# ubi-agni/mujoco_ros_pkgs

Measured on AMD Instinct MI355X. Metric: env_steps_per_sec, higher is better.
Workload: dtype f64

## Files before the change

### mujoco_ros_pkgs_amd/csrc/lane_env_topos.h

```cpp
#pragma once

struct LeTopo_franka_like {
	static constexpr const char *name = "franka_like";
	static constexpr int NBODY = 12;
	static constexpr int NQ = 9;
	static constexpr int NV = 9;
	static constexpr int NU = 9;
	static constexpr int NA = 0;
	static constexpr int NJNT = 9;
	static constexpr int NSITE = 1;
	static constexpr int NSENSOR = 20;
	static constexpr int NSENSORDATA = 25;
	static constexpr int NM = 44;
	static constexpr int body_parentid[12] = { 0, 0, 1, 2, 3, 4, 5, 6, 7, 8, 9, 9 };
	static constexpr int body_rootid[12] = { 0, 1, 1, 1, 1, 1, 1, 1, 1, 1, 1, 1 };
	static constexpr int body_jnt[12] = { -1, -1, 0, 1, 2, 3, 4, 5, 6, -1, 7, 8 };
	static constexpr int body_sameframe[12] = { 1, 0, 0, 0, 0, 0, 0, 0, 0, 0, 0, 0 };
	static constexpr int body_gc[12] = { 0, 0, 0, 0, 0, 0, 0, 0, 0, 0, 0, 0 };
	static constexpr int jnt_type[9] = { 3, 3, 3, 3, 3, 3, 3, 2, 2 };
	static constexpr int jnt_bodyid[9] = { 2, 3, 4, 5, 6, 7, 8, 10, 11 };
	static constexpr int dof_parentid[9] = { -1, 0, 1, 2, 3, 4, 5, 6, 6 };
	static constexpr int dof_Madr[9] = { 0, 1, 3, 6, 10, 15, 21, 28, 36 };
	static constexpr int act_jnt[9] = { 0, 1, 2, 3, 4, 5, 6, 7, 8 };
	static constexpr int act_gaintype[9] = { 0, 0, 0, 0, 0, 0, 0, 0, 0 };
	static constexpr int act_biastype[9] = { 0, 0, 0, 0, 0, 0, 0, 0, 0 };
	static constexpr int act_ctrllimited[9] = { 1, 1, 1, 1, 1, 1, 1, 1, 1 };
	static constexpr int act_forcelimited[9] = { 0, 0, 0, 0, 0, 0, 0, 0, 0 };
	static constexpr int act_dyntype[9] = { 0, 0, 0, 0, 0, 0, 0, 0, 0 };
	static constexpr int act_actadr[9] = { 0, 0, 0, 0, 0, 0, 0, 0, 0 };
	static constexpr int act_actlimited[9] = { 0, 0, 0, 0, 0, 0, 0, 0, 0 };
	static constexpr int site_bodyid[1] = { 9 };
	static constexpr int site_sameframe[1] = { 0 };
	static constexpr int sensor_type[20] = { 8, 8, 8, 8, 8, 8, 8, 8, 8, 9, 9, 9, 9, 9, 9, 9, 9, 9, 23, 24 };
	static constexpr int sensor_objtype[20] = { 3, 3, 3, 3, 3, 3, 3, 3, 3, 3, 3, 3, 3, 3, 3, 3, 3, 3, 6, 6 };
	static constexpr int sensor_objid[20] = { 0, 1, 2, 3, 4, 5, 6, 7, 8, 0, 1, 2, 3, 4, 5, 6, 7, 8, 0, 0 };
	static constexpr int sensor_adr[20] = { 0, 1, 2, 3, 4, 5, 6, 7, 8, 9, 10, 11, 12, 13, 14, 15, 16, 17, 18, 21 };
};

struct LeTopo_lane_env_tree {
	static constexpr const char *name = "lane_env_tree";
	static constexpr int NBODY = 10;
	static constexpr int NQ = 8;
	static constexpr int NV = 8;
	static constexpr int NU = 7;
	static constexpr int NA = 0;
	static constexpr int NJNT = 8;
	static constexpr int NSITE = 2;
	static constexpr int NSENSOR = 12;
	static constexpr int NSENSORDATA = 24;
	static constexpr int NM = 17;
	static constexpr int body_parentid[10] = { 0, 0, 1, 2, 1, 4, 5, 5, 0, 8 };
	static constexpr int body_rootid[10] = { 0, 1, 1, 1, 1, 1, 1, 1, 8, 8 };
	static constexpr int body_jnt[10] = { -1, 0, 1, 2, -1, 3, 4, 5, 6, 7 };
	static constexpr int body_sameframe[10] = { 1, 1, 0, 0, 0, 0, 0, 0, 0, 0 };
	static constexpr int body_gc[10] = { 0, 0, 0, 0, 0, 0, 0, 0, 0, 0 };
	static constexpr int jnt_type[8] = { 3, 3, 2, 3, 3, 2, 3, 3 };
	static constexpr int jnt_bodyid[8] = { 1, 2, 3, 5, 6, 7, 8, 9 };
	static constexpr int dof_parentid[8] = { -1, 0, 1, 0, 3, 3, -1, 6 };
	static constexpr int dof_Madr[8] = { 0, 1, 3, 6, 8, 11, 14, 15 };
	static constexpr int act_jnt[7] = { 0, 1, 2, 3, 4, 5, 6 };
	static constexpr int act_gaintype[7] = { 0, 0, 0, 0, 0, 0, 0 };
	static constexpr int act_biastype[7] = { 0, 0, 1, 0, 0, 1, 0 };
	static constexpr int act_ctrllimited[7] = { 1, 1, 1, 0, 0, 0, 1 };
	static constexpr int act_forcelimited[7] = { 0, 0, 0, 1, 0, 0, 0 };
	static constexpr int act_dyntype[7] = { 0, 0, 0, 0, 0, 0, 0 };
	static constexpr int act_actadr[7] = { 0, 0, 0, 0, 0, 0, 0 };
	static constexpr int act_actlimited[7] = { 0, 0, 0, 0, 0, 0, 0 };
	static constexpr int site_bodyid[2] = { 3, 7 };
	static constexpr int site_sameframe[2] = { 0, 0 };
	static constexpr int sensor_type[12] = { 8, 9, 14, 12, 13, 23, 24, 23, 24, 23, 35, 8 };
	static constexpr int sensor_objtype[12] = { 3, 3, 18, 18, 18, 6, 6, 6, 1, 2, 0, 3 };
	static constexpr int sensor_objid[12] = { 1, 4, 2, 2, 5, 0, 0, 1, 6, 9, -1, 7 };
	static constexpr int sensor_adr[12] = { 0, 1, 2, 3, 4, 5, 8, 12, 15, 19, 22, 23 };
};

#define MJB_LE_TOPOS(X) X(0, LeTopo_franka_like) X(1, LeTopo_lane_env_tree)
#define MJB_LE_NTOPO 2
```

### mujoco_ros_pkgs_amd/csrc/mjb_lane_env.hip

```cpp
#include <hip/hip_runtime.h>

#include <dlfcn.h>
#include <sys/stat.h>
#include <unistd.h>

#include <cstdio>
#include <cstdlib>

#include <atomic>
#include <map>
#include <mutex>
#include <string>
#include <vector>

#include "mjb_lane_env_kernel.h"
#include "lane_env_topos.h"

namespace {

using namespace mjb_le;

template <class T, int LP, bool PE = false, bool HW = false, bool XF = false>
__global__ void __launch_bounds__(64) mjb_lane_env_kernel(const KernelParams MJB_AS4 *__restrict__ P, const int nsteps, const unsigned int step0,
                                                          const int env_lo, const int env_hi)
{
	extern __shared__ __attribute__((aligned(16))) unsigned char smem_le[];
	lane_env_body<T, LP, LE_SOLO, PE, HW, XF>(P, nsteps, step0, env_lo, env_hi, smem_le);
}

template <class T, int LP>
__global__ void __launch_bounds__(128) mjb_lane_env_duo_kernel(const KernelParams MJB_AS4 *__restrict__ P, const int nsteps, const unsigned int step0,
                                                               const int env_lo, const int env_hi)
{
	extern __shared__ __attribute__((aligned(16))) unsigned char smem_le[];
	lane_env_duo<T, LP>(P, nsteps, step0, env_lo, env_hi, smem_le);
}

template <class T>
__global__ void __launch_bounds__(128) mjb_lane_env_duo2_kernel(const KernelParams MJB_AS4 *__restrict__ P, const int nsteps, const unsigned int step0,
                                                                const int env_lo, const int env_hi)
{
	extern __shared__ __attribute__((aligned(16))) unsigned char smem_le[];
	lane_env_duo2<T, 160>(P, nsteps, step0, env_lo, env_hi, smem_le);
}

template <class T, int NW>
__global__ void __launch_bounds__(64 * NW) mjb_lane_env_trio_kernel(const KernelParams MJB_AS4 *__restrict__ P, const int nsteps, const unsigned int step0,
                                                                    const int env_lo, const int env_hi)
{
	extern __shared__ __attribute__((aligned(16))) unsigned char smem_le[];
	if constexpr (NW == 4) lane_env_quartet<T, 160>(P, nsteps, step0, env_lo, env_hi, smem_le);
	else lane_env_trio<T, 160>(P, nsteps, step0, env_lo, env_hi, smem_le);
}

template <class T> bool topo_matches(const mjb_model_desc &h)
{
	if (h.nbody != T::NBODY || h.nq != T::NQ || h.nv != T::NV || h.nu != T::NU || h.na != T::NA || h.njnt != T::NJNT || h.nsite != T::NSITE ||
	    h.nsensor != T::NSENSOR || h.nsensordata != T::NSENSORDATA || h.nM != T::NM)
		return false;
	for (int b = 0; b < h.nbody; b++) {
		const int jn = h.body_jntnum[b] == 1 ? h.body_jntadr[b] : -1;
		if (h.body_jntnum[b] > 1 || h.body_parentid[b] != T::body_parentid[b] || h.body_rootid[b] != T::body_rootid[b] || jn != T::body_jnt[b] ||
		    (h.body_sameframe[b] != 0) != (T::body_sameframe[b] != 0))
			return false;
	}
	for (int j = 0; j < h.njnt; j++)
		if (h.jnt_type[j] != T::jnt_type[j] || h.jnt_bodyid[j] != T::jnt_bodyid[j] || h.jnt_qposadr[j] != j || h.jnt_dofadr[j] != j) return false;
	for (int d = 0; d < h.nv; d++)
		if (h.dof_parentid[d] != T::dof_parentid[d] || h.dof_Madr[d] != T::dof_Madr[d] || h.dof_jntid[d] != d) return false;
	for (int i = 0; i < h.nu; i++)
		if (h.actuator_trntype[i] != MJB_TRN_JOINT || h.actuator_dyntype[i] != T::act_dyntype[i] || h.actuator_trnid[2 * i] != T::act_jnt[i] ||
		    h.actuator_gaintype[i] != T::act_gaintype[i] || h.actuator_biastype[i] != T::act_biastype[i] ||
		    (h.actuator_ctrllimited[i] != 0) != (T::act_ctrllimited[i] != 0) || (h.actuator_forcelimited[i] != 0) != (T::act_forcelimited[i] != 0) ||
		    (h.na > 0 && (h.actuator_actadr[i] != T::act_actadr[i] || (h.actuator_actlimited[i] != 0) != (T::act_actlimited[i] != 0))))
			return false;
	for (int i = 0; i < h.nsite; i++)
		if (h.site_bodyid[i] != T::site_bodyid[i] || (h.site_sameframe[i] != 0) != (T::site_sameframe[i] != 0)) return false;
	for (int i = 0; i < h.nsensor; i++)
		if (h.sensor_type[i] != T::sensor_type[i] || h.sensor_objtype[i] != T::sensor_objtype[i] || h.sensor_objid[i] != T::sensor_objid[i] ||
		    h.sensor_adr[i] != T::sensor_adr[i] || h.sensor_refid[i] >= 0)
			return false;
	return true;
}

}

static bool le_plain_tree(const mjb_model_desc *h)
{
	return h && h->nefcmax <= 0 && h->nconmax <= 0 && h->integrator == MJB_INT_EULER && h->nmocap <= 0 && h->ntendon <= 0 && h->neq <= 0 &&
	       h->nq == h->nv && h->njnt == h->nv;
}
static bool le_dyntype_ok(const mjb_model_desc *h, int i)
{
	const int d = h->actuator_dyntype[i];
	if (d == MJB_DYN_NONE) return h->na <= 0 || h->actuator_actadr[i] < 0;
	return (d == MJB_DYN_INTEGRATOR || d == MJB_DYN_FILTER) && h->actuator_actadr[i] >= 0 && h->actuator_actadr[i] < h->na;
}

int mjb_lane_env_match(const mjb_model_desc *h)
{
	if (!le_plain_tree(h)) return -1;
	for (int b = 1; b < h->nbody; b++)
		if (h->body_gravcomp[b] != 0) return -1;
#define MJB_LE_X(id, T) \
	if (topo_matches<T>(*h)) return id;
	MJB_LE_TOPOS(MJB_LE_X)
#undef MJB_LE_X
	return -1;
}

namespace {
struct LeVariant {
	int form;
	int sweep;
	int lds_kb;
	LeBuild build;
	int wave_lanes;
	const char *unavailable;
};
struct LeRow {
// ... 19 lines not shown
		if (r.form == form && r.sweep == sweep && r.build == build) return &r;
	return nullptr;
}
constexpr int le_block(const LeVariant &v) { return v.form == 3 ? 64 * v.sweep : (v.form ? 128 : v.wave_lanes); }
template <class T, int LP> constexpr int le_lds_bytes(int form, int sweep)
{
	return form == 3 ? (sweep == 4 ? quartet_bytes<T>() : trio_bytes<T>()) : (form == 2 ? duo2_bytes<T>() : (form == 1 ? duo_bytes<T, LP>() : Lds<T, LP>::bytes()));
}
}


int mjb_lane_env_eligible(const mjb_model_desc *h)
{
	if (!le_plain_tree(h) || h->nv < 1 || h->nbody > 24 || h->nv > 20) return 0;
	for (int j = 0; j < h->njnt; j++)
		if ((h->jnt_type[j] != MJB_JNT_SLIDE && h->jnt_type[j] != MJB_JNT_HINGE) || h->jnt_qposadr[j] != j || h->jnt_dofadr[j] != j || h->dof_jntid[j] != j) return 0;
	for (int b = 0; b < h->nbody; b++)
		if (h->body_jntnum[b] > 1) return 0;
	for (int i = 0; i < h->nsensor; i++) {
		const int t = h->sensor_type[i], ot = h->sensor_objtype[i];
		const bool frame = t == MJB_SENS_FRAMEPOS || t == MJB_SENS_FRAMEQUAT;
		if (!(frame || t == MJB_SENS_JOINTPOS || t == MJB_SENS_JOINTVEL || t == MJB_SENS_ACTUATORFRC || t == MJB_SENS_ACTUATORPOS || t == MJB_SENS_ACTUATORVEL ||
		      t == MJB_SENS_CLOCK))
			return 0;
		if (frame && (h->sensor_refid[i] >= 0 || (ot != MJB_OBJ_BODY && ot != MJB_OBJ_XBODY && ot != MJB_OBJ_SITE))) return 0;
	}
	for (int i = 0; i < h->nu; i++)
		if (h->actuator_trntype[i] != MJB_TRN_JOINT || !le_dyntype_ok(h, i)) return 0;
	int owned = 0;
	for (int i = 0; i < h->nu; i++) owned += h->actuator_dyntype[i] != MJB_DYN_NONE;
	return owned == (h->na > 0 ? h->na : 0);
}

namespace {

std::string topo_source(const mjb_model_desc &h)
{
	std::string s = "struct LeTopo_rt {\n";
	auto scalar = [&](const char *n, int v) { s += std::string("\tstatic constexpr int ") + n + " = " + std::to_string(v) + ";\n"; };
	auto arr = [&](const char *n, int count, auto get) {
		s += std::string("\tstatic constexpr int ") + n + "[" + std::to_string(count > 0 ? count : 1) + "] = { ";
		for (int i = 0; i < (count > 0 ? count : 1); i++) s += (i ? ", " : "") + std::to_string(count > 0 ? (int)get(i) : 0);
		s += " };\n";
	};
	scalar("NBODY", h.nbody); scalar("NQ", h.nq); scalar("NV", h.nv); scalar("NU", h.nu); scalar("NA", h.na); scalar("NJNT", h.njnt); scalar("NSITE", h.nsite);
	scalar("NSENSOR", h.nsensor); scalar("NSENSORDATA", h.nsensordata); scalar("NM", h.nM);
	arr("body_parentid", h.nbody, [&](int i) { return h.body_parentid[i]; });
	arr("body_rootid", h.nbody, [&](int i) { return h.body_rootid[i]; });
	arr("body_jnt", h.nbody, [&](int i) { return h.body_jntnum[i] == 1 ? h.body_jntadr[i] : -1; });
	arr("body_sameframe", h.nbody, [&](int i) { return h.body_sameframe[i] != 0; });
	arr("body_gc", h.nbody, [&](int i) { return i > 0 && h.body_gravcomp[i] != 0; });
	arr("jnt_type", h.njnt, [&](int i) { return h.jnt_type[i]; });
	arr("jnt_bodyid", h.njnt, [&](int i) { return h.jnt_bodyid[i]; });
	arr("dof_parentid", h.nv, [&](int i) { return h.dof_parentid[i]; });
	arr("dof_Madr", h.nv, [&](int i) { return h.dof_Madr[i]; });
	arr("act_jnt", h.nu, [&](int i) { return h.actuator_trnid[2 * i]; });
	arr("act_gaintype", h.nu, [&](int i) { return h.actuator_gaintype[i]; });
	arr("act_biastype", h.nu, [&](int i) { return h.actuator_biastype[i]; });
	arr("act_ctrllimited", h.nu, [&](int i) { return h.actuator_ctrllimited[i] != 0; });
	arr("act_forcelimited", h.nu, [&](int i) { return h.actuator_forcelimited[i] != 0; });
	arr("act_dyntype", h.nu, [&](int i) { return h.actuator_dyntype[i]; });
	arr("act_actadr", h.nu, [&](int i) { return h.na > 0 ? h.actuator_actadr[i] : 0; });
	arr("act_actlimited", h.nu, [&](int i) { return h.na > 0 && h.actuator_actlimited[i] != 0; });
	arr("site_bodyid", h.nsite, [&](int i) { return h.site_bodyid[i]; });
	arr("site_sameframe", h.nsite, [&](int i) { return h.site_sameframe[i] != 0; });
	arr("sensor_type", h.nsensor, [&](int i) { return h.sensor_type[i]; });
	arr("sensor_objtype", h.nsensor, [&](int i) { return h.sensor_objtype[i]; });
	arr("sensor_objid", h.nsensor, [&](int i) { return h.sensor_objid[i]; });
	arr("sensor_adr", h.nsensor, [&](int i) { return h.sensor_adr[i]; });
	s += "};\n";
	return s;
}

struct RtcApi {
	void *lib = nullptr;
	int (*create)(void **, const char *, const char *, int, const char **, const char **) = nullptr;
	int (*compile)(void *, int, const char **) = nullptr;
	int (*log_size)(void *, size_t *) = nullptr;
	int (*log)(void *, char *) = nullptr;
	int (*code_size)(void *, size_t *) = nullptr;
	int (*code)(void *, char *) = nullptr;
	int (*destroy)(void **) = nullptr;
	bool ok = false;
};
RtcApi &rtc()
{
	static RtcApi a = [] {
		RtcApi r;
		for (const char *n : { "libhiprtc.so", "libhiprtc.so.7", "/opt/rocm/lib/libhiprtc.so" }) {
			r.lib = dlopen(n, RTLD_NOW | RTLD_LOCAL);
			if (r.lib) break;
		}
		if (!r.lib) return r;
		r.create = (decltype(r.create))dlsym(r.lib, "hiprtcCreateProgram");
		r.compile = (decltype(r.compile))dlsym(r.lib, "hiprtcCompileProgram");
		r.log_size = (decltype(r.log_size))dlsym(r.lib, "hiprtcGetProgramLogSize");
		r.log = (decltype(r.log))dlsym(r.lib, "hiprtcGetProgramLog");
		r.code_size = (decltype(r.code_size))dlsym(r.lib, "hiprtcGetCodeSize");
		r.code = (decltype(r.code))dlsym(r.lib, "hiprtcGetCode");
		r.destroy = (decltype(r.destroy))dlsym(r.lib, "hiprtcDestroyProgram");
		r.ok = r.create && r.compile && r.log_size && r.log && r.code_size && r.code && r.destroy;
		return r;
	}();
	return a;
}

// ... 529 lines not shown
```

### mujoco_ros_pkgs_amd/csrc/mjb_lane_env_kernel.h

```cpp
#pragma once
#ifndef __HIPCC_RTC__
#include <hip/hip_runtime.h>
#endif

#include "mjb_dev.h"
#include "mjb_math.h"

namespace mjb_le {

template <int V> struct IC {
	static constexpr int value = V;
	constexpr operator int() const { return V; }
};
template <int... Is> struct ISeq {};
template <int N, int... Is> struct MkSeq : MkSeq<N - 1, N - 1, Is...> {};
template <int... Is> struct MkSeq<0, Is...> { using type = ISeq<Is...>; };
template <typename F, int... Is> DEVI void sfor_impl(F &&f, ISeq<Is...>) { (f(IC<Is>{}), ...); }
template <int N, typename F> DEVI void sfor(F &&f) { sfor_impl(f, typename MkSeq<N>::type{}); }

DEVI double frcp(double x)
{
	double r = __builtin_amdgcn_rcp(x);
	r = fma(fma(-x, r, 1.0), r, r);
	r = fma(fma(-x, r, 1.0), r, r);
// ... 168 lines not shown
template <class T, int LP> struct Lds {
	using Q = Tq<T>;
	static constexpr bool needed(int b)
	{
		for (int a = b; a > 0; a = T::body_parentid[a])
			if (T::body_jnt[a] >= 0) return true;
		return false;
	}
	static constexpr int slot(int b)
	{
		int n = 0;
		for (int a = 1; a < b; a++)
			if (needed(a)) n++;
		return T::NV + 3 * n;
	}
	static constexpr int cin_slot(int b)
	{
		int at = slot(T::NBODY);
		for (int a = T::NBODY - 1; a >= 1; a--) {
			if (!needed(a)) continue;
			if (at + 5 > LP) return -1;
			if (a == b) return at;
			at += 5;
		}
		return -1;
	}
	static constexpr int nmov() { return (slot(T::NBODY) - T::NV) / 3; }
	static constexpr int nslots() { return le_solo_slots(T::NV, nmov(), LP); }
	static constexpr int bytes() { return nslots() * LE_SLOT_BYTES; }
};

struct alignas(16) Pair { double a, b; };

template <class T> struct PeSlots {
	static constexpr bool moving(int b) { return Lds<T, (1 << 20)>::needed(b); }
	static constexpr int njb(int b) { int n = 0; for (int a = 1; a < b; a++) if (T::body_jnt[a] >= 0) n++; return n; }
	static constexpr int nmb(int b) { int n = 0; for (int a = 1; a < b; a++) if (moving(a)) n++; return n; }
	static constexpr int gravity(int k) { return k; }
	static constexpr int joint(int b, int f) { return 3 + 4 * njb(b) + f; }
	static constexpr int inert(int b, int f) { return 3 + 4 * njb(T::NBODY) + 7 * nmb(b) + f; }
	static constexpr int act(int i, int f) { return 3 + 4 * njb(T::NBODY) + 7 * nmb(T::NBODY) + 6 * i + f; }
	static constexpr int rest(int b) { return act(T::NU, 0) + (b - 1 - nmb(b)); }
	static constexpr int n = act(T::NU, 0) + (T::NBODY - 1 - nmb(T::NBODY));
};

template <class T> struct XfSlots {
	static constexpr int slot(int b) { return PeSlots<T>::nmb(b); }
	static constexpr int n = PeSlots<T>::nmb(T::NBODY);
};

template <class T, class = void> struct LeGc { static constexpr bool on(int) { return false; } };
template <class T> struct LeGc<T, decltype((void)T::body_gc)> { static constexpr bool on(int b) { return T::body_gc[b] != 0; } };
template <class T> constexpr bool le_any_gc() { for (int b = 1; b < T::NBODY; b++) if (LeGc<T>::on(b)) return true; return false; }

enum LeRole : int {
	LE_SOLO = 0,
	LE_DUO_P = 1,
	LE_DUO_V = 2,
	LE_PIPE_P = 3,
	LE_PIPE_V = 4,
	LE_TRIO_P = 5,
	LE_TRIO_C = 6,
	LE_TRIO_V = 7,
	LE_QUAD_O = 8,
	LE_QUAD_X = 9,
	LE_QUAD_C = 10,
	LE_QUAD_V = 11,
};
constexpr bool le_two_halves(int role) { return role == LE_DUO_P || role == LE_DUO_V; }
constexpr bool le_pipelined_duo(int role) { return role == LE_PIPE_P || role == LE_PIPE_V; }
constexpr bool le_trio(int role) { return role == LE_TRIO_P || role == LE_TRIO_C || role == LE_TRIO_V; }
constexpr bool le_quartet(int role) { return role == LE_QUAD_O || role == LE_QUAD_X || role == LE_QUAD_C || role == LE_QUAD_V; }
DEVI void le_barrier() { asm volatile("s_waitcnt lgkmcnt(0)\n\ts_barrier" ::: "memory"); }
template <int NV> struct DuoSlots { static constexpr int n = le_exchange_slots(NV); };
template <class T, int LP, int ROLE = LE_SOLO, bool PE = false, bool HW = false, bool XF = false>
DEVI void lane_env_body(const KernelParams MJB_AS4 *__restrict__ P, const int nsteps, const unsigned int step0, const int env_lo, const int env_hi,
                        unsigned char *const smem_le)
{
	constexpr int NB = T::NBODY, NV = T::NV, NU = T::NU, NA = T::NA;
	constexpr bool QUAD = le_quartet(ROLE), TRIQ = le_trio(ROLE) || QUAD;
	constexpr bool HALVES = ROLE == LE_SOLO || le_two_halves(ROLE);
	constexpr bool DP = ROLE == LE_SOLO || ROLE == LE_DUO_P || ROLE == LE_PIPE_P || ROLE == LE_TRIO_C || ROLE == LE_QUAD_C, DV = ROLE == LE_SOLO || ROLE == LE_DUO_V || ROLE == LE_PIPE_V || ROLE == LE_TRIO_V || ROLE == LE_QUAD_V, DUO = ROLE != LE_SOLO;
	constexpr bool PIPE = le_pipelined_duo(ROLE) || TRIQ;
	constexpr bool POSE = HALVES || ROLE == LE_PIPE_P || ROLE == LE_TRIO_P, RINGC = ROLE == LE_PIPE_V || ROLE == LE_TRIO_C || ROLE == LE_TRIO_V;
	constexpr bool VLDS = ROLE == LE_TRIO_V || ROLE == LE_QUAD_V;
	constexpr bool EPOS = ROLE == LE_SOLO || ROLE == LE_DUO_P || ROLE == LE_PIPE_P || ROLE == LE_TRIO_P || ROLE == LE_QUAD_X;
	constexpr bool SENSF = ROLE == LE_SOLO || ROLE == LE_DUO_V || ROLE == LE_PIPE_P || ROLE == LE_TRIO_P || ROLE == LE_QUAD_X;
	[[maybe_unused]] constexpr bool XW = ROLE == LE_QUAD_X;
	[[maybe_unused]] constexpr bool DPW = DP || XW;
	[[maybe_unused]] constexpr bool FM = ROLE != LE_QUAD_C, FH = !XW;
	[[maybe_unused]] constexpr bool POSEW = ROLE == LE_TRIO_P || ROLE == LE_QUAD_X;
	[[maybe_unused]] constexpr bool OWNCIN = ROLE != LE_TRIO_V;
	using Q = Tq<T>;
	static_assert(!PE || ROLE == LE_SOLO, "lane = env kernel: per-env overrides run the solo form");
	static_assert(!HW || (ROLE == LE_SOLO && !PE), "lane = env kernel: the hwsim stage runs the solo form, without per-env overrides");
	static_assert(!XF || (ROLE == LE_SOLO && !HW), "lane = env kernel: xfrc_applied runs the solo form, without the hwsim stage");
	static_assert(NA == 0 || (ROLE == LE_SOLO && !HW), "lane = env kernel: activation states run the solo form, without the hwsim stage");
	static_assert(!le_any_gc<T>() || ROLE == LE_SOLO, "lane = env kernel: gravity compensation runs the solo form");
	using OV = PeSlots<T>;
	using XS6 = XfSlots<T>;
	constexpr int LPE = PIPE ? (1 << 20) : (DUO ? LP - DuoSlots<NV>::n : LP);
	using LD = Lds<T, LPE>;
	static_assert(LD::slot(T::NBODY) <= LPE, "lane = env kernel: state and forces of the topology need more LDS than this instantiation's budget");
	constexpr auto SCUSE = [](int b) {
		if (b < 3 || b >= T::NBODY || T::body_jnt[b] < 0) return false;
		if (T::jnt_type[T::body_jnt[b]] != MJB_JNT_HINGE) return false;
// ... 266 lines not shown
						matvec3(v, xm, ip);
						for (int k = 0; k < 3; k++) dif[k] += v[k];
					}
					const double mass = tj.mass;
					const double *X = xm;
					const double ixx = tj.ibody[0], iyy = tj.ibody[1], izz = tj.ibody[2], ixy = tj.ibody[3], ixz = tj.ibody[4], iyz = tj.ibody[5];
					double Tm[9];
					for (int rr = 0; rr < 3; rr++) {
						Tm[3 * rr + 0] = X[3 * rr] * ixx + X[3 * rr + 1] * ixy + X[3 * rr + 2] * ixz;
						Tm[3 * rr + 1] = X[3 * rr] * ixy + X[3 * rr + 1] * iyy + X[3 * rr + 2] * iyz;
						Tm[3 * rr + 2] = X[3 * rr] * ixz + X[3 * rr + 1] * iyz + X[3 * rr + 2] * izz;
					}
					ci[0] = Tm[0] * X[0] + Tm[1] * X[1] + Tm[2] * X[2] + mass * (dif[1] * dif[1] + dif[2] * dif[2]);
					ci[1] = Tm[3] * X[3] + Tm[4] * X[4] + Tm[5] * X[5] + mass * (dif[0] * dif[0] + dif[2] * dif[2]);
					ci[2] = Tm[6] * X[6] + Tm[7] * X[7] + Tm[8] * X[8] + mass * (dif[0] * dif[0] + dif[1] * dif[1]);
					ci[3] = Tm[0] * X[3] + Tm[1] * X[4] + Tm[2] * X[5] - mass * dif[0] * dif[1];
					ci[4] = Tm[0] * X[6] + Tm[1] * X[7] + Tm[2] * X[8] - mass * dif[0] * dif[2];
					ci[5] = Tm[3] * X[6] + Tm[4] * X[7] + Tm[5] * X[8] - mass * dif[1] * dif[2];
					ci[6] = mass * dif[0];
					ci[7] = mass * dif[1];
					ci[8] = mass * dif[2];
					ci[9] = mass;
					if constexpr (OWNCIN) for (int k = 0; k < 5; k++) lp[64 * (c0 + k)] = Pair{ ci[2 * k], ci[2 * k + 1] };
				}
				[[maybe_unused]] double pv[6], pa[6];
				if constexpr (!DV) {
				} else if constexpr (p == 0 || !LD::needed(p)) {
					for (int k = 0; k < 6; k++) pv[k] = 0;
					pa[0] = pa[1] = pa[2] = 0;
					for (int k = 0; k < 3; k++) pa[3 + k] = -grav[k];
				} else {
					for (int k = 0; k < 6; k++) { pv[k] = cvel[p][k]; pa[k] = cacc[p][k]; }
				}
				if constexpr (j >= 0) {
					[[maybe_unused]] double qv = 0;
					if constexpr (DV) qv = lp[64 * j].b;
					double *cd = cdof[j];
					constexpr int cq = CD0 + 3 * (ord % 2);
					if constexpr (ROLE == LE_QUAD_V) {
						const Pair d0 = lp[64 * cq], d1 = lp[64 * (cq + 1)], d2 = lp[64 * (cq + 2)];
						cd[0] = d0.a; cd[1] = d0.b; cd[2] = d1.a; cd[3] = d1.b; cd[4] = d2.a; cd[5] = d2.b;
						if constexpr (T::jnt_type[j] == MJB_JNT_SLIDE) cd[0] = cd[1] = cd[2] = 0;
					} else {
					const LeTapeBody MJB_AS4 &tj = tb[b];
					const double ax[3] = { tj.jaxis[0], tj.jaxis[1], tj.jaxis[2] };
					double xaxis[3];
					matvec3(xaxis, xm, ax);
					if constexpr (T::jnt_type[j] == MJB_JNT_SLIDE) {
						cd[0] = cd[1] = cd[2] = 0;
						for (int k = 0; k < 3; k++) cd[3 + k] = xaxis[k];
					} else {
						const double jp[3] = { tj.jpos[0], tj.jpos[1], tj.jpos[2] };
						double xanch[3] = { xp[0], xp[1], xp[2] }, off[3];
						if (jp[0] != 0 || jp[1] != 0 || jp[2] != 0) {
							double v[3];
							matvec3(v, xm, jp);
							for (int k = 0; k < 3; k++) xanch[k] += v[k];
						}
						for (int k = 0; k < 3; k++) off[k] = -xanch[k];
						for (int k = 0; k < 3; k++) cd[k] = xaxis[k];
						cross3(cd + 3, xaxis, off);
					}
					if constexpr (ROLE == LE_QUAD_C) {
						lp[64 * cq] = Pair{ cd[0], cd[1] };
						lp[64 * (cq + 1)] = Pair{ cd[2], cd[3] };
						lp[64 * (cq + 2)] = Pair{ cd[4], cd[5] };
					}
					}
					if constexpr (!DV) {
					} else if constexpr (p == 0 || !LD::needed(p)) {
						for (int k = 0; k < 6; k++) { cvel[b][k] = cd[k] * qv; cacc[b][k] = pa[k]; }
					} else {
						double cdd[6];
						cross_motion(cdd, pv, cd);
						for (int k = 0; k < 6; k++) { cvel[b][k] = pv[k] + cd[k] * qv; cacc[b][k] = pa[k] + cdd[k] * qv; }
					}
				} else if constexpr (DV) {
					for (int k = 0; k < 6; k++) { cvel[b][k] = pv[k]; cacc[b][k] = pa[k]; }
				}
				if constexpr (DV) {
					double cf[6], t0[6], t1[6];
					mul_inert_vec(cf, ci, cacc[b]);
					mul_inert_vec(t0, ci, cvel[b]);
					cross_force(t1, cvel[b], t0);
					constexpr int q0 = LD::slot(b);
					lp[64 * q0] = Pair{ cf[0] + t1[0], cf[1] + t1[1] };
					lp[64 * (q0 + 1)] = Pair{ cf[2] + t1[2], cf[3] + t1[3] };
					lp[64 * (q0 + 2)] = Pair{ cf[4] + t1[4], cf[5] + t1[5] };
				}
			};
			[[maybe_unused]] double hcmd[NV > 0 ? NV : 1], hpi[NV > 0 ? NV : 1], hpl[NV > 0 ? NV : 1], hjp[NV > 0 ? NV : 1], hjv[NV > 0 ? NV : 1], hlu = 0, hlw = 0;
			[[maybe_unused]] auto hw_fetch = [&]() __attribute__((always_inline)) {
				if (Pq->hw.period_ns > 0) {
					const double *const cad = Pq->hw.cad + ev * (size_t)(2 + 2 * Pq->hw.n);
					hlu = cad[0];
					hlw = cad[1];
				}
				sfor<NV>([&](auto I) __attribute__((always_inline)) {
					hcmd[I] = hpi[I] = hpl[I] = hjp[I] = hjv[I] = 0;
					const HwSim MJB_AS4 &hw = Pq->hw;
					const int k = hw.le_tab[4 * I];
					if (k >= 0) {
						const int method = hw.le_tab[4 * I + 1], hn = hw.n;
						const size_t at = ev * (size_t)hn + (size_t)k;
						if (method == MJB_HW_EFFORT) hcmd[I] = hw.cmd_eff[at];
						else if (method == MJB_HW_VELOCITY || method == MJB_HW_VELOCITY_PID) hcmd[I] = hw.cmd_vel[at];
						else if (hw.estop != 0) hcmd[I] = hw.cmd_hold[at];
// ... 227 lines not shown
						}
						constexpr int q0 = LD::slot(b);
						lp[64 * q0] = Pair{ cf[0] + t1[0], cf[1] + t1[1] };
						lp[64 * (q0 + 1)] = Pair{ cf[2] + t1[2], cf[3] + t1[3] };
						lp[64 * (q0 + 2)] = Pair{ cf[4] + t1[4], cf[5] + t1[5] };
					}
					if constexpr (ROLE == LE_PIPE_P || ROLE == LE_TRIO_P) {
						constexpr int ord = (LD::slot(b) - NV) / 3, rg = RING + 6 * (ord % RINGN);
						const double *xm = xmat[b];
						double xp[3] = { 0, 0, 0 };
						if constexpr (r != b) for (int k = 0; k < 3; k++) xp[k] = xpos[b][k] - xpos[r][k];
						lp[64 * rg] = Pair{ xp[0], xp[1] };
						lp[64 * (rg + 1)] = Pair{ xp[2], xm[0] };
						lp[64 * (rg + 2)] = Pair{ xm[1], xm[2] };
						lp[64 * (rg + 3)] = Pair{ xm[3], xm[4] };
						lp[64 * (rg + 4)] = Pair{ xm[5], xm[6] };
						lp[64 * (rg + 5)] = Pair{ xm[7], xm[8] };
						LE_PK(0);
						le_barrier();
						LE_PK(2);
					}
				}
				if constexpr (b + 1 < NB) touch_rec<14>(hA[b + 1]);
				if constexpr (DV && b == NB - 1) sfor<NV>([&](auto I) { qfa[I] = s.qfrc_applied[ev * NV + I]; });
				if constexpr (HW && b == NB - 1) hw_fetch();
				__builtin_amdgcn_sched_barrier(0);
				}
			});


			if constexpr (QUAD) {
				constexpr auto HINGE = [](int c) {
					if (c < 1 || c >= T::NBODY || T::body_jnt[c < T::NBODY ? (c < 0 ? 0 : c) : 0] < 0) return false;
					return T::jnt_type[T::body_jnt[c]] == MJB_JNT_HINGE;
				};
				constexpr auto NEXTN = [](int c) { for (int q = c + 1; q < T::NBODY; q++) if (LD::needed(q)) return q; return T::NBODY; };
				constexpr auto NTH = [](int k) { int c = 0; for (int i = 0; i < k && c < T::NBODY; i++) { c++; while (c < T::NBODY && !LD::needed(c)) c++; } return k < 1 ? T::NBODY : c; };
				constexpr int KN = [] { int n = 0; for (int c = 1; c < T::NBODY; c++) if (LD::needed(c)) n++; return n; }();
				constexpr int N1 = NEXTN(0), N2 = NEXTN(N1 < NB ? N1 : NB - 1);
				[[maybe_unused]] double osn[NB + 1], ocs[NB + 1], oq0[NB + 1];
				[[maybe_unused]] Pair opq[NB + 1];
				auto o_body = [&](auto Bq) {
					constexpr int b = Bq;
					constexpr int p = T::body_parentid[b], j = T::body_jnt[b];
					const double *const A = hA[b];
					constexpr int qr = QR0 + 4 * (((LD::slot(b) - NV) / 3) % 2);
					double quat[4] = { A[3], A[4], A[5], A[6] };
					if constexpr (p != 0) {
						double q[4];
						qmul(q, xquat[p], quat);
						for (int k = 0; k < 4; k++) quat[k] = q[k];
					}
					if constexpr (j >= 0) {
						if (A[10] != 0 || A[11] != 0 || A[12] != 0) {
							lp[64 * (qr + 2)] = Pair{ quat[0], quat[1] };
							lp[64 * (qr + 3)] = Pair{ quat[2], quat[3] };
						}
						if constexpr (T::jnt_type[j] == MJB_JNT_HINGE) {
							double ql[4], q[4];
							ql[0] = ocs[b]; ql[1] = A[7] * osn[b]; ql[2] = A[8] * osn[b]; ql[3] = A[9] * osn[b];
							qmul(q, quat, ql);
							for (int k = 0; k < 4; k++) quat[k] = q[k];
						}
					}
					normalize4_sel(quat);
					for (int k = 0; k < 4; k++) xquat[b][k] = quat[k];
					if constexpr (LD::needed(b)) {
						lp[64 * qr] = Pair{ quat[0], quat[1] };
						lp[64 * (qr + 1)] = Pair{ quat[2], quat[3] };
					}
				};
				auto o_phase = [&](auto Bq) {
					constexpr int b = Bq, nx = NEXTN(b), nx2 = NEXTN(nx < NB ? nx : NB - 1);
					touch_s(hA[b][0]);
					if constexpr (nx < NB) for (int k = 0; k < 14; k++) hA[nx][k] = reinterpret_cast<const double MJB_AS4 *>(tb + nx)[k];
					if constexpr (nx < NB && HINGE(nx2)) {
						opq[nx2] = lp[64 * T::body_jnt[nx2 < NB ? nx2 : 0]];
						oq0[nx2] = tb[nx2].qpos0;
					}
					if constexpr (HINGE(nx)) sincos_nb((opq[nx].a - oq0[nx]) * 0.5, &osn[nx], &ocs[nx]);
					o_body(Bq);
					if constexpr (nx < NB) touch_rec<14>(hA[nx]);
				};
				auto x_body = [&](auto Bq) {
					constexpr int b = Bq;
					constexpr int p = T::body_parentid[b], j = T::body_jnt[b], r = T::body_rootid[b];
					constexpr int qr = QR0 + 4 * (((LD::slot(b) - NV) / 3) % 2);
					const double *const A = hA[b];
					double pos[3] = { A[0], A[1], A[2] }, quat[4] = { A[3], A[4], A[5], A[6] };
					if constexpr (LD::needed(b)) {
						const Pair g0 = lp[64 * qr], g1 = lp[64 * (qr + 1)];
						quat[0] = g0.a; quat[1] = g0.b; quat[2] = g1.a; quat[3] = g1.b;
					} else {
						if constexpr (p != 0) {
							double q[4];
							qmul(q, xquat[p], quat);
							for (int k = 0; k < 4; k++) quat[k] = q[k];
						}
						normalize4_sel(quat);
					}
					[[maybe_unused]] Pair sp{ 0, 0 };
					if constexpr (j >= 0) sp = lp[64 * j];
					if constexpr (p != 0) {
						double v[3];
						matvec3(v, xmat[p], pos);
						for (int k = 0; k < 3; k++) pos[k] = v[k] + xpos[p][k];
					}
					[[maybe_unused]] double xanch[3], qp = 0;
					[[maybe_unused]] bool offc = false;
					if constexpr (j >= 0) {
						qp = sp.a;
						const double jp[3] = { A[10], A[11], A[12] };
						offc = jp[0] != 0 || jp[1] != 0 || jp[2] != 0;
						for (int k = 0; k < 3; k++) xanch[k] = pos[k];
						if (offc) {
							const Pair h0 = lp[64 * (qr + 2)], h1 = lp[64 * (qr + 3)];
							const double q0[4] = { h0.a, h0.b, h1.a, h1.b };
							double M0[9], v[3];
							quat2mat_nocheck(M0, q0);
							matvec3(v, M0, jp);
							for (int k = 0; k < 3; k++) xanch[k] += v[k];
						}
						if (ep_on && pas_on) {
							const double dqs = qp - tb[b].spring;
							pe += 0.5 * tb[b].stiffness * dqs * dqs;
						}
					}
					for (int k = 0; k < 4; k++) xquat[b][k] = quat[k];
					quat2mat_nocheck(xmat[b], quat);
					if constexpr (j >= 0) {
						if constexpr (T::jnt_type[j] == MJB_JNT_SLIDE) {
							const double ax[3] = { A[7], A[8], A[9] };
							double xaxis[3];
							matvec3(xaxis, xmat[b], ax);
							const double dq = qp - A[13];
							for (int k = 0; k < 3; k++) pos[k] += xaxis[k] * dq;
						} else if (offc) {
							const double jp[3] = { A[10], A[11], A[12] };
							double v[3];
							matvec3(v, xmat[b], jp);
							for (int k = 0; k < 3; k++) pos[k] = xanch[k] - v[k];
						}
					}
					for (int k = 0; k < 3; k++) xpos[b][k] = pos[k];
					const double *const Bh = hB[b];
					double xipos[3];
					if constexpr (T::body_sameframe[b]) {
						for (int k = 0; k < 3; k++) xipos[k] = xpos[b][k];
					} else {
						double ip[3] = { Bh[0], Bh[1], Bh[2] }, v[3];
						matvec3(v, xmat[b], ip);
						for (int k = 0; k < 3; k++) xipos[k] = v[k] + xpos[b][k];
					}
					if (eg_on) pe -= Bh[9] * (grav[0] * xipos[0] + grav[1] * xipos[1] + grav[2] * xipos[2]);
					frame_sensors(Bq, xipos);
					if constexpr (LD::needed(b)) {
						constexpr int ord = (LD::slot(b) - NV) / 3, rg = RING + 6 * (ord % RINGN);
						const double *xm = xmat[b];
						double xp[3] = { 0, 0, 0 };
						if constexpr (r != b) for (int k = 0; k < 3; k++) xp[k] = xpos[b][k] - xpos[r][k];
						lp[64 * rg] = Pair{ xp[0], xp[1] };
						lp[64 * (rg + 1)] = Pair{ xp[2], xm[0] };
						lp[64 * (rg + 2)] = Pair{ xm[1], xm[2] };
						lp[64 * (rg + 3)] = Pair{ xm[3], xm[4] };
						lp[64 * (rg + 4)] = Pair{ xm[5], xm[6] };
						lp[64 * (rg + 5)] = Pair{ xm[7], xm[8] };
						if constexpr (j >= 0) {
							double *cd = cdof[j];
							const double ax[3] = { A[7], A[8], A[9] };
							double xaxis[3];
							matvec3(xaxis, xm, ax);
							if constexpr (T::jnt_type[j] == MJB_JNT_SLIDE) {
								cd[0] = cd[1] = cd[2] = 0;
								for (int k = 0; k < 3; k++) cd[3 + k] = xaxis[k];
							} else {
								const double jp[3] = { A[10], A[11], A[12] };
								double xa[3] = { xp[0], xp[1], xp[2] }, off[3];
								if (jp[0] != 0 || jp[1] != 0 || jp[2] != 0) {
									double v[3];
									matvec3(v, xm, jp);
									for (int k = 0; k < 3; k++) xa[k] += v[k];
								}
								for (int k = 0; k < 3; k++) off[k] = -xa[k];
								for (int k = 0; k < 3; k++) cd[k] = xaxis[k];
								cross3(cd + 3, xaxis, off);
							}
						}
					}
				};
				auto x_phase = [&](auto Bq) {
					constexpr int b = Bq, nx = NEXTN(b);
					touch_s(hA[b][0]);
					touch_s(hB[b][0]);
					if constexpr (nx < NB) {
						for (int k = 0; k < 14; k++) hA[nx][k] = reinterpret_cast<const double MJB_AS4 *>(tb + nx)[k];
						for (int k = 0; k < 10; k++) hB[nx][k] = reinterpret_cast<const double MJB_AS4 *>(tb + nx)[16 + k];
					}
					x_body(Bq);
					if constexpr (nx < NB) {
						touch_rec<14>(hA[nx]);
						touch_rec<10>(hB[nx]);
					}
				};
				if constexpr (ROLE == LE_QUAD_O || ROLE == LE_QUAD_X) {
					sfor<NB>([&](auto Bq) {
						constexpr int b = Bq;
						if constexpr (b > 0 && !LD::needed(b)) {
							for (int k = 0; k < 14; k++) hA[b][k] = reinterpret_cast<const double MJB_AS4 *>(tb + b)[k];
							if constexpr (ROLE == LE_QUAD_X) for (int k = 0; k < 10; k++) hB[b][k] = reinterpret_cast<const double MJB_AS4 *>(tb + b)[16 + k];
							if constexpr (ROLE == LE_QUAD_O) o_body(Bq);
							else x_body(Bq);
						}
					});
					if constexpr (N1 < NB) {
						for (int k = 0; k < 14; k++) hA[N1][k] = reinterpret_cast<const double MJB_AS4 *>(tb + N1)[k];
						if constexpr (ROLE == LE_QUAD_X) for (int k = 0; k < 10; k++) hB[N1][k] = reinterpret_cast<const double MJB_AS4 *>(tb + N1)[16 + k];
					}
					if constexpr (ROLE == LE_QUAD_O) {
						if constexpr (HINGE(N1)) {
							opq[N1] = lp[64 * T::body_jnt[N1 < NB ? N1 : 0]];
							oq0[N1] = tb[N1].qpos0;
						}
						if constexpr (N1 < NB && HINGE(N2)) {
							opq[N2] = lp[64 * T::body_jnt[N2 < NB ? N2 : 0]];
							oq0[N2] = tb[N2].qpos0;
						}
						if constexpr (HINGE(N1)) sincos_nb((opq[N1].a - oq0[N1]) * 0.5, &osn[N1], &ocs[N1]);
					}
				}
				__builtin_amdgcn_sched_barrier(0);
				sfor<KN + 3>([&](auto Ki) {
					constexpr int k = Ki + 1;
					constexpr int kk = k - (ROLE - LE_QUAD_O);
					if constexpr (kk >= 1 && kk <= KN) {
						constexpr int bb = NTH(kk);
						if constexpr (ROLE == LE_QUAD_O) o_phase(IC<bb>{});
						else if constexpr (ROLE == LE_QUAD_X) x_phase(IC<bb>{});
						else consume(IC<bb>{});
					}
					if constexpr (DV && k == 1) sfor<NV>([&](auto I) { qfa[I] = s.qfrc_applied[ev * NV + I]; });
					if constexpr (k <= KN + 2) {
						LE_PK(0);
						le_barrier();
						LE_PK(2);
					}
					__builtin_amdgcn_sched_barrier(0);
				});
			}

			LE_PK(0);
			if constexpr (TRIQ && !QUAD) {
				le_barrier();
				if constexpr (ROLE == LE_TRIO_V) consume(IC<LASTB>{});
			}
			LE_PK(1);
			if constexpr (DV) {
				if (nz_on && attempt == 0) {
					const double rate = Pq->nz.rate, scale = Pq->nz.scale;
					sfor<NU>([&](auto I) { const double v = rate * cn[I] + scale * z[I]; cn[I] = rs ? 0.0 : v; });
				}
				double ctrl[NU > 0 ? NU : 1];
				if (nz_on) {
					sfor<NU>([&](auto I) { ctrl[I] = cn[I]; });
				} else {
					sfor<NU>([&](auto I) { const double c = pinv(s.ctrl[ev * NU + I]); ctrl[I] = wasreset ? 0.0 : c; });
				}
				[[maybe_unused]] bool h_upd = false, h_wr = false;
				[[maybe_unused]] double h_dt = dt;
				[[maybe_unused]] const bool h_run = attempt == 0 || hw_bad;
				if constexpr (HW) {
					const HwSim MJB_AS4 &hw = Pq->hw;
					const long long per_ns = hw.period_ns;
					h_wr = true;
					if (per_ns > 0) {
						const double lu0 = pinv(hlu), lw0 = pinv(hlw);
						const long long t = ros_ns_nb(time);
						long long lu = (long long)lu0, lw = (long long)lw0;
						const bool back = t < lu;
						lu = sell(back, t, lu);
						lw = sell(back, t, lw);
						const long long sim_period = t - lu;
						h_upd = (sim_period >= per_ns) | ((lu == 0) & (sim_period != 0));
						lu = sell(h_upd, t, lu);
						h_wr = (lu != 0) & (t > lw);
						h_dt = 1e-9 * (double)(t - lw);
						double *const cad = hw.cad + ev * (size_t)(2 + 2 * hw.n);
						const double lu1 = (double)lu, lw1 = (double)sell(h_wr, t, lw);
						cad[0] = seld(h_run, lu1, lu0);
						cad[1] = seld(h_run, lw1, lw0);
					}
					h_upd = h_upd & h_run;
					hw_wr = (h_run & h_wr) | (!h_run & hw_wr);
// ... 550 lines not shown
```

Before: 547.9 million.

## Specialize joint-offset checks at compile time and reuse staged cdof in quad X role

Adds a per-topology compile-time table saying whether each joint has a nonzero position offset, and validates it against the model at dispatch. Kernels use it to drop the runtime jpos tests and, in the prefetch touch, skip scalar register pins for fields that are never read. The X role in the quad pipeline no longer recomputes cdof from the rotation matrix. It copies cdof values already staged in LDS by another wave, three phases later. This cuts ALU and SGPR pressure on the critical path, but relies on the LDS slot layout and a deferred read timing that must line up with the producer.

```diff
diff --git a/mujoco_ros_pkgs_amd/csrc/lane_env_topos.h b/mujoco_ros_pkgs_amd/csrc/lane_env_topos.h
--- a/mujoco_ros_pkgs_amd/csrc/lane_env_topos.h
+++ b/mujoco_ros_pkgs_amd/csrc/lane_env_topos.h
@@ -19,6 +19,7 @@
 	static constexpr int body_gc[12] = { 0, 0, 0, 0, 0, 0, 0, 0, 0, 0, 0, 0 };
 	static constexpr int jnt_type[9] = { 3, 3, 3, 3, 3, 3, 3, 2, 2 };
 	static constexpr int jnt_bodyid[9] = { 2, 3, 4, 5, 6, 7, 8, 10, 11 };
+	static constexpr int jnt_offc[9] = { 0, 0, 0, 0, 0, 0, 0, 0, 0 };
 	static constexpr int dof_parentid[9] = { -1, 0, 1, 2, 3, 4, 5, 6, 6 };
 	static constexpr int dof_Madr[9] = { 0, 1, 3, 6, 10, 15, 21, 28, 36 };
 	static constexpr int act_jnt[9] = { 0, 1, 2, 3, 4, 5, 6, 7, 8 };
@@ -56,6 +57,7 @@
 	static constexpr int body_gc[10] = { 0, 0, 0, 0, 0, 0, 0, 0, 0, 0 };
 	static constexpr int jnt_type[8] = { 3, 3, 2, 3, 3, 2, 3, 3 };
 	static constexpr int jnt_bodyid[8] = { 1, 2, 3, 5, 6, 7, 8, 9 };
+	static constexpr int jnt_offc[8] = { 1, 1, 1, 0, 1, 0, 0, 1 };
 	static constexpr int dof_parentid[8] = { -1, 0, 1, 0, 3, 3, -1, 6 };
 	static constexpr int dof_Madr[8] = { 0, 1, 3, 6, 8, 11, 14, 15 };
 	static constexpr int act_jnt[7] = { 0, 1, 2, 3, 4, 5, 6 };
diff --git a/mujoco_ros_pkgs_amd/csrc/mjb_lane_env.hip b/mujoco_ros_pkgs_amd/csrc/mjb_lane_env.hip
--- a/mujoco_ros_pkgs_amd/csrc/mjb_lane_env.hip
+++ b/mujoco_ros_pkgs_amd/csrc/mjb_lane_env.hip
@@ -52,6 +52,8 @@
 	if constexpr (NW == 4) lane_env_quartet<T, 160>(P, nsteps, step0, env_lo, env_hi, smem_le);
 	else lane_env_trio<T, 160>(P, nsteps, step0, env_lo, env_hi, smem_le);
 }
+
+static bool le_jnt_offc(const mjb_model_desc &h, int j) { return h.jnt_pos[3 * j] != 0 || h.jnt_pos[3 * j + 1] != 0 || h.jnt_pos[3 * j + 2] != 0; }
 
 template <class T> bool topo_matches(const mjb_model_desc &h)
 {
@@ -66,6 +68,9 @@
 	}
 	for (int j = 0; j < h.njnt; j++)
 		if (h.jnt_type[j] != T::jnt_type[j] || h.jnt_bodyid[j] != T::jnt_bodyid[j] || h.jnt_qposadr[j] != j || h.jnt_dofadr[j] != j) return false;
+	if constexpr (LeOffc<T>::known)
+		for (int j = 0; j < h.njnt; j++)
+			if (le_jnt_offc(h, j) != LeOffc<T>::on(j)) return false;
 	for (int d = 0; d < h.nv; d++)
 		if (h.dof_parentid[d] != T::dof_parentid[d] || h.dof_Madr[d] != T::dof_Madr[d] || h.dof_jntid[d] != d) return false;
 	for (int i = 0; i < h.nu; i++)
@@ -191,6 +196,7 @@
 	arr("body_gc", h.nbody, [&](int i) { return i > 0 && h.body_gravcomp[i] != 0; });
 	arr("jnt_type", h.njnt, [&](int i) { return h.jnt_type[i]; });
 	arr("jnt_bodyid", h.njnt, [&](int i) { return h.jnt_bodyid[i]; });
+	arr("jnt_offc", h.njnt, [&](int i) { return le_jnt_offc(h, i); });
 	arr("dof_parentid", h.nv, [&](int i) { return h.dof_parentid[i]; });
 	arr("dof_Madr", h.nv, [&](int i) { return h.dof_Madr[i]; });
 	arr("act_jnt", h.nu, [&](int i) { return h.actuator_trnid[2 * i]; });
diff --git a/mujoco_ros_pkgs_amd/csrc/mjb_lane_env_kernel.h b/mujoco_ros_pkgs_amd/csrc/mjb_lane_env_kernel.h
--- a/mujoco_ros_pkgs_amd/csrc/mjb_lane_env_kernel.h
+++ b/mujoco_ros_pkgs_amd/csrc/mjb_lane_env_kernel.h
@@ -244,6 +244,14 @@
 template <class T, class = void> struct LeGc { static constexpr bool on(int) { return false; } };
 template <class T> struct LeGc<T, decltype((void)T::body_gc)> { static constexpr bool on(int b) { return T::body_gc[b] != 0; } };
 template <class T> constexpr bool le_any_gc() { for (int b = 1; b < T::NBODY; b++) if (LeGc<T>::on(b)) return true; return false; }
+
+template <class T, class = void> struct LeOffc { static constexpr bool known = false; static constexpr bool on(int) { return false; } };
+template <class T> struct LeOffc<T, decltype((void)T::jnt_offc)> { static constexpr bool known = true; static constexpr bool on(int j) { return T::jnt_offc[j] != 0; } };
+template <class T, bool USE, int J> DEVI bool le_offc(const double jx, const double jy, const double jz)
+{
+	if constexpr (USE && LeOffc<T>::known) return LeOffc<T>::on(J);
+	else return jx != 0 || jy != 0 || jz != 0;
+}
 
 enum LeRole : int {
 	LE_SOLO = 0,
@@ -616,7 +624,7 @@
 					} else {
 						const double jp[3] = { tj.jpos[0], tj.jpos[1], tj.jpos[2] };
 						double xanch[3] = { xp[0], xp[1], xp[2] }, off[3];
-						if (jp[0] != 0 || jp[1] != 0 || jp[2] != 0) {
+						if (le_offc<T, QUAD, j>(jp[0], jp[1], jp[2])) {
 							double v[3];
 							matvec3(v, xm, jp);
 							for (int k = 0; k < 3; k++) xanch[k] += v[k];
@@ -950,7 +958,7 @@
 						for (int k = 0; k < 4; k++) quat[k] = q[k];
 					}
 					if constexpr (j >= 0) {
-						if (A[10] != 0 || A[11] != 0 || A[12] != 0) {
+						if (le_offc<T, true, j>(A[10], A[11], A[12])) {
 							lp[64 * (qr + 2)] = Pair{ quat[0], quat[1] };
 							lp[64 * (qr + 3)] = Pair{ quat[2], quat[3] };
 						}
@@ -1009,7 +1017,7 @@
 					if constexpr (j >= 0) {
 						qp = sp.a;
 						const double jp[3] = { A[10], A[11], A[12] };
-						offc = jp[0] != 0 || jp[1] != 0 || jp[2] != 0;
+						offc = le_offc<T, true, j>(jp[0], jp[1], jp[2]);
 						for (int k = 0; k < 3; k++) xanch[k] = pos[k];
 						if (offc) {
 							const Pair h0 = lp[64 * (qr + 2)], h1 = lp[64 * (qr + 3)];
@@ -1063,27 +1071,16 @@
 						lp[64 * (rg + 3)] = Pair{ xm[3], xm[4] };
 						lp[64 * (rg + 4)] = Pair{ xm[5], xm[6] };
 						lp[64 * (rg + 5)] = Pair{ xm[7], xm[8] };
-						if constexpr (j >= 0) {
-							double *cd = cdof[j];
-							const double ax[3] = { A[7], A[8], A[9] };
-							double xaxis[3];
-							matvec3(xaxis, xm, ax);
-							if constexpr (T::jnt_type[j] == MJB_JNT_SLIDE) {
-								cd[0] = cd[1] = cd[2] = 0;
-								for (int k = 0; k < 3; k++) cd[3 + k] = xaxis[k];
-							} else {
-								const double jp[3] = { A[10], A[11], A[12] };
-								double xa[3] = { xp[0], xp[1], xp[2] }, off[3];
-								if (jp[0] != 0 || jp[1] != 0 || jp[2] != 0) {
-									double v[3];
-									matvec3(v, xm, jp);
-									for (int k = 0; k < 3; k++) xa[k] += v[k];
-								}
-								for (int k = 0; k < 3; k++) off[k] = -xa[k];
-								for (int k = 0; k < 3; k++) cd[k] = xaxis[k];
-								cross3(cd + 3, xaxis, off);
-							}
-						}
+					}
+				};
+				[[maybe_unused]] auto x_cdof = [&](auto Bq) {
+					constexpr int b = Bq, j = T::body_jnt[b];
+					if constexpr (j >= 0) {
+						constexpr int cq = CD0 + 3 * (((LD::slot(b) - NV) / 3) % 2);
+						const Pair d0 = lp[64 * cq], d1 = lp[64 * (cq + 1)], d2 = lp[64 * (cq + 2)];
+						double *cd = cdof[j];
+						cd[0] = d0.a; cd[1] = d0.b; cd[2] = d1.a; cd[3] = d1.b; cd[4] = d2.a; cd[5] = d2.b;
+						if constexpr (T::jnt_type[j] == MJB_JNT_SLIDE) cd[0] = cd[1] = cd[2] = 0;
 					}
 				};
 				auto x_phase = [&](auto Bq) {
@@ -1096,8 +1093,14 @@
 					}
 					x_body(Bq);
 					if constexpr (nx < NB) {
-						touch_rec<14>(hA[nx]);
-						touch_rec<10>(hB[nx]);
+						constexpr int jn = T::body_jnt[nx];
+						const double *const a = hA[nx], *const h = hB[nx];
+						asm volatile("" ::"s"(a[0]), "s"(a[1]), "s"(a[2]), "s"(h[9]));
+						if constexpr (!T::body_sameframe[nx]) asm volatile("" ::"s"(h[0]), "s"(h[1]), "s"(h[2]));
+						if constexpr (jn >= 0) {
+							if constexpr (T::jnt_type[jn < 0 ? 0 : jn] == MJB_JNT_SLIDE) asm volatile("" ::"s"(a[7]), "s"(a[8]), "s"(a[9]), "s"(a[13]));
+							if constexpr (!LeOffc<T>::known || LeOffc<T>::on(jn < 0 ? 0 : jn)) asm volatile("" ::"s"(a[10]), "s"(a[11]), "s"(a[12]));
+						}
 					}
 				};
 				if constexpr (ROLE == LE_QUAD_O || ROLE == LE_QUAD_X) {
@@ -1136,6 +1139,7 @@
 						else if constexpr (ROLE == LE_QUAD_X) x_phase(IC<bb>{});
 						else consume(IC<bb>{});
 					}
+					if constexpr (ROLE == LE_QUAD_X && k - 3 >= 1 && k - 3 <= KN) x_cdof(IC<NTH(k - 3 >= 1 ? k - 3 : 1)>{});
 					if constexpr (DV && k == 1) sfor<NV>([&](auto I) { qfa[I] = s.qfrc_applied[ev * NV + I]; });
 					if constexpr (k <= KN + 2) {
 						LE_PK(0);
```

Result: faster. 604.2 million (median of 6 runs) (+10.3%).
